# microsoft/XPretrain

Hardware: NVIDIA H100
Metric: video-text pairs/sec (12f x 224^2, 32 tok), CLIP-ViP ViT-B/16 fwd+InfoNCE+bwd (higher is better)
Workload: dtype bf16

## Files before the change

### xpretrain_b200/csrc/attn_wgmma.cuh

```cuda
#pragma once
#include "ptx.cuh"
#include "mma_frag.cuh"

namespace xp {

constexpr int ATILE = 64;
constexpr int ATILE_BYTES = ATILE * 128;
constexpr int STREAM_THREADS = 384;

constexpr int stream_fwd_smem(int stages) { return (2 + 2 * stages) * ATILE_BYTES + 1024 + 64; }
constexpr int stream_kv_smem(int stages) { return (4 + 2 * stages) * ATILE_BYTES + stages * 2 * ATILE * 4 + 1024 + 64; }
constexpr int stream_q_smem(int stages) { return (4 + 2 * stages) * ATILE_BYTES + 1024 + 64; }

__device__ __forceinline__ uint64_t kdesc(uint32_t addr) { return make_smem_desc_sw128(addr, 16, 1024); }
__device__ __forceinline__ uint64_t mndesc(uint32_t addr) { return make_smem_desc_sw128(addr, 8192, 1024); }

__device__ __forceinline__ void acc_to_afrag(const float (&x)[32], uint32_t (&a)[4][4]) {
#pragma unroll
  for (int ks = 0; ks < 4; ++ks) {
    a[ks][0] = pack_bf16(x[8 * ks + 0], x[8 * ks + 1]);
    a[ks][1] = pack_bf16(x[8 * ks + 2], x[8 * ks + 3]);
    a[ks][2] = pack_bf16(x[8 * ks + 4], x[8 * ks + 5]);
    a[ks][3] = pack_bf16(x[8 * ks + 6], x[8 * ks + 7]);
  }
}

template <class Live>
__device__ __forceinline__ void fwd_step(uint32_t sQ, uint32_t sK, uint32_t sV, float (&o)[32], float (&m_run)[2],
                                         float (&l_run)[2], Live live, bool partial = true) {
  const int lane = threadIdx.x & 31, q_lo = ((threadIdx.x >> 5) & 3) * 16 + (lane >> 2);
  float s[32];
#pragma unroll
  for (int i = 0; i < 32; ++i) s[i] = 0.f;
  wgmma_fence_regs(s);
  wgmma_fence();
#pragma unroll
  for (int ks = 0; ks < 4; ++ks) wgmma_m64n64k16_ss<0, 0>(s, kdesc(sQ + ks * 32), kdesc(sK + ks * 32));
  wgmma_commit();
  wgmma_wait<0>();
  wgmma_fence_regs(s);
  if (partial) {
#pragma unroll
    for (int i = 0; i < 8; ++i)
#pragma unroll
      for (int e = 0; e < 4; ++e)
        if (!live(q_lo + (e >> 1) * 8, i * 8 + (lane & 3) * 2 + (e & 1))) s[4 * i + e] = -INFINITY;
  }
// ... 30 lines not shown
    for (int j = 0; j < 4; ++j)
      pl[ks][j] = pack_bf16(s[8 * ks + 2 * j] - bf16_lo(ph[ks][j]), s[8 * ks + 2 * j + 1] - bf16_hi(ph[ks][j]));
  wgmma_fence_regs(o);
  wgmma_fence();
#pragma unroll
  for (int ks = 0; ks < 4; ++ks) {
    const uint64_t vd = mndesc(sV + ks * 16 * 128);
    wgmma_m64n64k16_rs<1>(o, ph[ks], vd);
    wgmma_m64n64k16_rs<1>(o, pl[ks], vd);
  }
  wgmma_commit();
  wgmma_wait<0>();
  wgmma_fence_regs(o);
}

__device__ __forceinline__ void quad_sum(float (&l_run)[2]) {
#pragma unroll
  for (int r = 0; r < 2; ++r) {
    l_run[r] += __shfl_xor_sync(0xffffffffu, l_run[r], 1);
    l_run[r] += __shfl_xor_sync(0xffffffffu, l_run[r], 2);
  }
}

template <class Live>
__device__ __forceinline__ void kv_step(uint32_t sK, uint32_t sV, uint32_t sQ, uint32_t sdO, const float* s_lse,
                                        const float* s_delta, float (&dk)[32], float (&dv)[32], Live live) {
  const int lane = threadIdx.x & 31, k_lo = ((threadIdx.x >> 5) & 3) * 16 + (lane >> 2);
  float st[32], dpt[32];
#pragma unroll
  for (int i = 0; i < 32; ++i) st[i] = dpt[i] = 0.f;
  wgmma_fence_regs(st);
  wgmma_fence_regs(dpt);
  wgmma_fence();
#pragma unroll
  for (int ks = 0; ks < 4; ++ks) {
    wgmma_m64n64k16_ss<0, 0>(st, kdesc(sK + ks * 32), kdesc(sQ + ks * 32));
    wgmma_m64n64k16_ss<0, 0>(dpt, kdesc(sV + ks * 32), kdesc(sdO + ks * 32));
  }
  wgmma_commit();
  wgmma_wait<0>();
  wgmma_fence_regs(st);
  wgmma_fence_regs(dpt);
#pragma unroll
  for (int i = 0; i < 8; ++i)
#pragma unroll
    for (int e = 0; e < 4; ++e) {
      const int q = i * 8 + (lane & 3) * 2 + (e & 1);
      const float p = live(q, k_lo + (e >> 1) * 8) ? fast_exp2(fmaf(st[4 * i + e], LOG2E, -s_lse[q])) : 0.f;
      st[4 * i + e] = p;
      dpt[4 * i + e] = p * (dpt[4 * i + e] - s_delta[q]);
    }
  uint32_t ap[4][4], ad[4][4];
  acc_to_afrag(st, ap);
  acc_to_afrag(dpt, ad);
  wgmma_fence_regs(dv);
  wgmma_fence_regs(dk);
  wgmma_fence();
#pragma unroll
  for (int ks = 0; ks < 4; ++ks) {
    wgmma_m64n64k16_rs<1>(dv, ap[ks], mndesc(sdO + ks * 16 * 128));
    wgmma_m64n64k16_rs<1>(dk, ad[ks], mndesc(sQ + ks * 16 * 128));
  }
  wgmma_commit();
  wgmma_wait<0>();
  wgmma_fence_regs(dv);
  wgmma_fence_regs(dk);
}

template <class Live>
__device__ __forceinline__ void q_step(uint32_t sQ, uint32_t sdO, uint32_t sK, uint32_t sV, const float (&lse_r)[2],
                                       const float (&del_r)[2], float (&dq)[32], Live live) {
  const int lane = threadIdx.x & 31, q_lo = ((threadIdx.x >> 5) & 3) * 16 + (lane >> 2);
  float s[32], dp[32];
#pragma unroll
  for (int i = 0; i < 32; ++i) s[i] = dp[i] = 0.f;
  wgmma_fence_regs(s);
  wgmma_fence_regs(dp);
  wgmma_fence();
#pragma unroll
  for (int ks = 0; ks < 4; ++ks) {
    wgmma_m64n64k16_ss<0, 0>(s, kdesc(sQ + ks * 32), kdesc(sK + ks * 32));
    wgmma_m64n64k16_ss<0, 0>(dp, kdesc(sdO + ks * 32), kdesc(sV + ks * 32));
  }
  wgmma_commit();
  wgmma_wait<0>();
  wgmma_fence_regs(s);
  wgmma_fence_regs(dp);
#pragma unroll
  for (int i = 0; i < 8; ++i)
#pragma unroll
    for (int e = 0; e < 4; ++e) {
      const bool valid = live(q_lo + (e >> 1) * 8, i * 8 + (lane & 3) * 2 + (e & 1));
      const float p = valid ? fast_exp2(fmaf(s[4 * i + e], LOG2E, -lse_r[e >> 1])) : 0.f;
      dp[4 * i + e] = p * (dp[4 * i + e] - del_r[e >> 1]);
    }
  uint32_t ad[4][4];
  acc_to_afrag(dp, ad);
  wgmma_fence_regs(dq);
  wgmma_fence();
#pragma unroll
  for (int ks = 0; ks < 4; ++ks) wgmma_m64n64k16_rs<1>(dq, ad[ks], mndesc(sK + ks * 16 * 128));
  wgmma_commit();
  wgmma_wait<0>();
  wgmma_fence_regs(dq);
}

template <int STAGES>
__device__ __forceinline__ void init_ring(uint64_t* q_full, uint64_t* full, uint64_t* empty, uint32_t full_count,
                                          int nlive, const CUtensorMap* tm0, const CUtensorMap* tm1) {
  if (threadIdx.x == 0) {
    tma_prefetch_desc(tm0);
    tma_prefetch_desc(tm1);
    mbar_init(q_full, 1);
#pragma unroll
    for (int s = 0; s < STAGES; ++s) {
      mbar_init(&full[s], full_count);
      mbar_init(&empty[s], 4 * nlive);
    }
    fence_barrier_init();
  }
  __syncthreads();
}
__device__ __forceinline__ void release_stage(uint64_t* empty, int s) {
  __syncwarp();
// ... 197 lines not shown
```

### xpretrain_b200/csrc/common.cu

```cuda
#include "common.h"

#include <mutex>

#include "../../include/xpretrain_b200.h"

namespace xp {

static thread_local std::string t_error;
std::atomic<int64_t> g_launches{0};

void set_error(const std::string& msg) { t_error = msg; }
int fail(const std::string& msg) {
  t_error = msg;
  return -1;
}

int sm_count() {
  static int cached[64] = {0};
  int dev = 0;
  if (cudaGetDevice(&dev) != cudaSuccess || dev < 0 || dev >= 64) return 132;
  if (cached[dev] == 0) {
    int n = 0;
    if (cudaDeviceGetAttribute(&n, cudaDevAttrMultiProcessorCount, dev) != cudaSuccess || n <= 0) n = 132;
    cached[dev] = n;
// ... 76 lines not shown
                  CU_TENSOR_MAP_FLOAT_OOB_FILL_NONE);
  if (r != CUDA_SUCCESS) return fail("cuTensorMapEncodeTiled failed with CUresult " + std::to_string(int(r)));
  return 0;
}

int make_tmap_bf16_3d(CUtensorMap* out, const void* base, uint64_t inner, uint64_t mid, uint64_t outer,
                      uint64_t row_stride, uint64_t mid_stride, uint32_t box_inner, uint32_t box_mid) {
  EncodeTiledFn fn = encode_fn();
  if (!fn) return fail("cuTensorMapEncodeTiled unavailable (no CUDA driver / no GPU): this library has no CPU path");
  if (!aligned(base, 16)) return fail("tensor map: base pointer must be 16-byte aligned");
  if ((row_stride * 2) % 16 != 0 || (mid_stride * 2) % 16 != 0)
    return fail("tensor map: strides must be multiples of 8 bf16 elements");
  cuuint64_t dims[3] = {inner, mid, outer};
  cuuint64_t strides[2] = {row_stride * 2, mid_stride * 2};
  cuuint32_t box[3] = {box_inner, box_mid, 1};
  cuuint32_t estr[3] = {1, 1, 1};
  CUresult r = fn(out, CU_TENSOR_MAP_DATA_TYPE_BFLOAT16, 3, const_cast<void*>(base), dims, strides, box, estr,
                  CU_TENSOR_MAP_INTERLEAVE_NONE, CU_TENSOR_MAP_SWIZZLE_128B, CU_TENSOR_MAP_L2_PROMOTION_L2_256B,
                  CU_TENSOR_MAP_FLOAT_OOB_FILL_NONE);
  if (r != CUDA_SUCCESS) return fail("cuTensorMapEncodeTiled failed with CUresult " + std::to_string(int(r)));
  return 0;
}

}

extern "C" {
int xp_version(void) { return XP_ABI_VERSION; }
const char* xp_last_error(void) { return xp::t_error.c_str(); }
int64_t xp_launch_count(void) { return xp::g_launches.load(); }
void xp_launch_count_reset(void) { xp::g_launches.store(0); }
}
```

### xpretrain_b200/csrc/common.h

```cpp
#pragma once
#include <cuda.h>
#include <cuda_bf16.h>
#include <cuda_fp16.h>
#include <cuda_runtime.h>
#include <stdint.h>

#include <atomic>
#include <string>
#include <type_traits>

#include "../../include/xpretrain_b200.h"

namespace xp {

void set_error(const std::string& msg);
int fail(const std::string& msg);
extern std::atomic<int64_t> g_launches;
inline void count_launch(int n = 1) { g_launches.fetch_add(n, std::memory_order_relaxed); }

int sm_count();

int make_tmap_bf16_2d(CUtensorMap* out, const void* base, uint64_t inner, uint64_t outer, uint64_t row_stride,
                      uint32_t box_inner, uint32_t box_outer);
int make_tmap_bf16_3d(CUtensorMap* out, const void* base, uint64_t inner, uint64_t mid, uint64_t outer,
                      uint64_t row_stride, uint64_t mid_stride, uint32_t box_inner, uint32_t box_mid);

int ensure_context(const void* device_ptr);
#define XP_ENTER(ptr)                                   \
  do {                                                  \
    if (::xp::ensure_context(ptr) != 0) return -1;      \
  } while (0)

#define XP_CHECK_CUDA(expr)                                                                         \
  do {                                                                                              \
    cudaError_t _e = (expr);                                                                        \
    if (_e != cudaSuccess) return ::xp::fail(std::string(#expr) + ": " + cudaGetErrorString(_e)); \
  } while (0)

#define XP_CHECK_LAUNCH(name)                                                                             \
  do {                                                                                                    \
    cudaError_t _e = cudaGetLastError();                                                                  \
    if (_e != cudaSuccess) return ::xp::fail(std::string(name) + " launch: " + cudaGetErrorString(_e)); \
    ::xp::count_launch();                                                                                 \
  } while (0)

inline bool aligned(const void* p, uintptr_t bytes) { return (reinterpret_cast<uintptr_t>(p) & (bytes - 1)) == 0; }

template <auto K>
// ... 25 lines not shown
```

### xpretrain_b200/csrc/ptx.cuh

```cuda
#pragma once
#include <cuda.h>
#include <cuda_bf16.h>
#include <cuda_fp16.h>
#include <cuda_runtime.h>
#include <stdint.h>
#include <stdio.h>

namespace xp {

#ifndef XP_WAIT_TIMEOUT_CYCLES
#define XP_WAIT_TIMEOUT_CYCLES (8000000000ll)
#endif

__device__ __forceinline__ uint32_t smem_u32(const void* p) {
  return static_cast<uint32_t>(__cvta_generic_to_shared(p));
}
__device__ __forceinline__ int lane_id() { return threadIdx.x & 31; }

__device__ __forceinline__ void mbar_init(uint64_t* bar, uint32_t count) {
  asm volatile("mbarrier.init.shared::cta.b64 [%0], %1;" ::"r"(smem_u32(bar)), "r"(count) : "memory");
}
__device__ __forceinline__ void fence_barrier_init() {
  asm volatile("fence.mbarrier_init.release.cluster;" ::: "memory");
}
// ... 33 lines not shown
}
__device__ __forceinline__ void mbar_wait_nocall(uint64_t* bar, uint32_t parity) {
  if (mbar_try_wait(bar, parity)) return;
  long long t0 = clock64();
  while (!mbar_try_wait(bar, parity)) {
    if (clock64() - t0 > XP_WAIT_TIMEOUT_CYCLES) __trap();
  }
}

__device__ __forceinline__ void tma_prefetch_desc(const CUtensorMap* m) {
  asm volatile("prefetch.tensormap [%0];" ::"l"(reinterpret_cast<uint64_t>(m)) : "memory");
}
__device__ __forceinline__ void tma_load_2d(void* smem_dst, const CUtensorMap* m, uint64_t* bar, int c0, int c1) {
  asm volatile(
      "cp.async.bulk.tensor.2d.shared::cluster.global.mbarrier::complete_tx::bytes [%0], [%1, {%3, %4}], [%2];"
      ::"r"(smem_u32(smem_dst)), "l"(reinterpret_cast<uint64_t>(m)), "r"(smem_u32(bar)), "r"(c0), "r"(c1)
      : "memory");
}
__device__ __forceinline__ void tma_load_3d(void* smem_dst, const CUtensorMap* m, uint64_t* bar, int c0, int c1,
                                            int c2) {
  asm volatile(
      "cp.async.bulk.tensor.3d.shared::cluster.global.mbarrier::complete_tx::bytes [%0], [%1, {%3, %4, %5}], [%2];"
      ::"r"(smem_u32(smem_dst)), "l"(reinterpret_cast<uint64_t>(m)), "r"(smem_u32(bar)), "r"(c0), "r"(c1), "r"(c2)
      : "memory");
}

__device__ __forceinline__ void tma_store_2d(const CUtensorMap* m, uint32_t smem_src, int c0, int c1) {
  asm volatile("cp.async.bulk.tensor.2d.global.shared::cta.bulk_group [%0, {%2, %3}], [%1];" ::"l"(
                   reinterpret_cast<uint64_t>(m)),
               "r"(smem_src), "r"(c0), "r"(c1)
               : "memory");
}
__device__ __forceinline__ void tma_store_commit() { asm volatile("cp.async.bulk.commit_group;" ::: "memory"); }
template <int N>
__device__ __forceinline__ void tma_store_wait_read() {
  asm volatile("cp.async.bulk.wait_group.read %0;" ::"n"(N) : "memory");
}

__device__ __forceinline__ void wgmma_fence() { asm volatile("wgmma.fence.sync.aligned;" ::: "memory"); }
__device__ __forceinline__ void wgmma_commit() { asm volatile("wgmma.commit_group.sync.aligned;" ::: "memory"); }
template <int N>
__device__ __forceinline__ void wgmma_wait() {
  asm volatile("wgmma.wait_group.sync.aligned %0;" ::"n"(N) : "memory");
}
template <int R>
__device__ __forceinline__ void wgmma_fence_regs(float (&d)[R]) {
// ... 14 lines not shown
        "+f"(d[8]), "+f"(d[9]), "+f"(d[10]), "+f"(d[11]), "+f"(d[12]), "+f"(d[13]), "+f"(d[14]), "+f"(d[15]),
        "+f"(d[16]), "+f"(d[17]), "+f"(d[18]), "+f"(d[19]), "+f"(d[20]), "+f"(d[21]), "+f"(d[22]), "+f"(d[23]),
        "+f"(d[24]), "+f"(d[25]), "+f"(d[26]), "+f"(d[27]), "+f"(d[28]), "+f"(d[29]), "+f"(d[30]), "+f"(d[31]),
        "+f"(d[32]), "+f"(d[33]), "+f"(d[34]), "+f"(d[35]), "+f"(d[36]), "+f"(d[37]), "+f"(d[38]), "+f"(d[39]),
        "+f"(d[40]), "+f"(d[41]), "+f"(d[42]), "+f"(d[43]), "+f"(d[44]), "+f"(d[45]), "+f"(d[46]), "+f"(d[47]),
        "+f"(d[48]), "+f"(d[49]), "+f"(d[50]), "+f"(d[51]), "+f"(d[52]), "+f"(d[53]), "+f"(d[54]), "+f"(d[55]),
        "+f"(d[56]), "+f"(d[57]), "+f"(d[58]), "+f"(d[59]), "+f"(d[60]), "+f"(d[61]), "+f"(d[62]), "+f"(d[63])
      : "l"(adesc), "l"(bdesc), "n"(TA), "n"(TB));
}

template <int TA, int TB>
__device__ __forceinline__ void wgmma_m64n64k16_ss(float (&d)[32], uint64_t adesc, uint64_t bdesc) {
  asm volatile(
      "wgmma.mma_async.sync.aligned.m64n64k16.f32.bf16.bf16 {"
      "%0, %1, %2, %3, %4, %5, %6, %7, %8, %9, %10, %11, %12, %13, %14, %15, "
      "%16, %17, %18, %19, %20, %21, %22, %23, %24, %25, %26, %27, %28, %29, %30, %31"
      "}, %32, %33, 1, 1, 1, %34, %35;"
      : "+f"(d[0]), "+f"(d[1]), "+f"(d[2]), "+f"(d[3]), "+f"(d[4]), "+f"(d[5]), "+f"(d[6]), "+f"(d[7]),
        "+f"(d[8]), "+f"(d[9]), "+f"(d[10]), "+f"(d[11]), "+f"(d[12]), "+f"(d[13]), "+f"(d[14]), "+f"(d[15]),
        "+f"(d[16]), "+f"(d[17]), "+f"(d[18]), "+f"(d[19]), "+f"(d[20]), "+f"(d[21]), "+f"(d[22]), "+f"(d[23]),
        "+f"(d[24]), "+f"(d[25]), "+f"(d[26]), "+f"(d[27]), "+f"(d[28]), "+f"(d[29]), "+f"(d[30]), "+f"(d[31])
      : "l"(adesc), "l"(bdesc), "n"(TA), "n"(TB));
}
template <int TB>
__device__ __forceinline__ void wgmma_m64n64k16_rs(float (&d)[32], const uint32_t (&a)[4], uint64_t bdesc) {
  asm volatile(
      "wgmma.mma_async.sync.aligned.m64n64k16.f32.bf16.bf16 {"
      "%0, %1, %2, %3, %4, %5, %6, %7, %8, %9, %10, %11, %12, %13, %14, %15, "
      "%16, %17, %18, %19, %20, %21, %22, %23, %24, %25, %26, %27, %28, %29, %30, %31"
      "}, {%32, %33, %34, %35}, %36, 1, 1, 1, %37;"
      : "+f"(d[0]), "+f"(d[1]), "+f"(d[2]), "+f"(d[3]), "+f"(d[4]), "+f"(d[5]), "+f"(d[6]), "+f"(d[7]),
        "+f"(d[8]), "+f"(d[9]), "+f"(d[10]), "+f"(d[11]), "+f"(d[12]), "+f"(d[13]), "+f"(d[14]), "+f"(d[15]),
        "+f"(d[16]), "+f"(d[17]), "+f"(d[18]), "+f"(d[19]), "+f"(d[20]), "+f"(d[21]), "+f"(d[22]), "+f"(d[23]),
        "+f"(d[24]), "+f"(d[25]), "+f"(d[26]), "+f"(d[27]), "+f"(d[28]), "+f"(d[29]), "+f"(d[30]), "+f"(d[31])
      : "r"(a[0]), "r"(a[1]), "r"(a[2]), "r"(a[3]), "l"(bdesc), "n"(TB));
}

template <uint32_t N>
__device__ __forceinline__ void setmaxnreg_dec() {
  asm volatile("setmaxnreg.dec.sync.aligned.u32 %0;" ::"n"(N));
}
template <uint32_t N>
__device__ __forceinline__ void setmaxnreg_inc() {
  asm volatile("setmaxnreg.inc.sync.aligned.u32 %0;" ::"n"(N));
}
__device__ __forceinline__ void named_bar_sync(uint32_t id, uint32_t threads) {
// ... 130 lines not shown
```

### xpretrain_b200/csrc/vip_attention.cu

```cuda
#include "../../include/xpretrain_b200.h"
#include "common.h"
#include "attn_wgmma.cuh"
#include "vip_attention.h"

namespace xp {

constexpr int SROWS = 256;
constexpr int GROW = 248;
constexpr int MAT_BYTES = SROWS * 128;
constexpr int TILE_BYTES = 64 * 128;
constexpr int ATT_THREADS = 256;

__device__ __forceinline__ bool row_valid(int r, const AttnDims& d) { return r < d.L || (r >= GROW && r < GROW + d.M); }
__device__ __forceinline__ bool row_global(int r) { return r >= GROW; }
__device__ __forceinline__ int row_seq(int r, const AttnDims& d) { return r >= GROW ? r - GROW : d.M + r; }
__device__ __forceinline__ bool tile_live(int k, const AttnDims& d) { return k == 3 || 64 * k < d.L; }

template <int NMAT>
__device__ __forceinline__ void stage_rows(uint8_t* sm, uint64_t* bar, const CUtensorMap* const (&mapL)[NMAT],
                                           const CUtensorMap* const (&mapM)[NMAT], const int (&col)[NMAT], const AttnDims& d,
                                           int b, int t) {
  if (threadIdx.x == 0) {
    mbar_init(bar, 1);
    fence_barrier_init();
// ... 79 lines not shown
}

__global__ void __launch_bounds__(64)
vip_attn_fwd_combine_kernel(const float* __restrict__ part, __nv_bfloat16* __restrict__ out, float* __restrict__ lse,
                            const AttnDims d) {
  const int h = blockIdx.x, b = blockIdx.y, c = threadIdx.x;
  for (int m = 0; m < d.M; ++m) {
    const float* p0 = part + ((static_cast<long long>(b) * d.H + h) * d.T * d.M + m) * 66;
    float mx = -INFINITY;
    for (int t = 0; t < d.T; ++t) mx = fmaxf(mx, p0[static_cast<long long>(t) * d.M * 66]);
    float l = 0.f, acc = 0.f;
    for (int t = 0; t < d.T; ++t) {
      const float* p = p0 + static_cast<long long>(t) * d.M * 66;
      const float w = __expf(p[0] - mx);
      l += p[1] * w;
      acc += p[2 + c] * w;
    }
    out[(static_cast<long long>(b) * d.S + m) * d.ld_o + h * HD + c] = __float2bfloat16(acc / l);
    if (c == 0) lse[(static_cast<long long>(b) * d.H + h) * d.S + m] = mx + logf(l);
  }
}


__global__ void __launch_bounds__(ATT_THREADS, 1)
vip_attn_bwd_kernel(const __grid_constant__ CUtensorMap tmL, const __grid_constant__ CUtensorMap tmM,
                    const __grid_constant__ CUtensorMap tdL, const __grid_constant__ CUtensorMap tdM,
                    const __nv_bfloat16* __restrict__ out, const __nv_bfloat16* __restrict__ dout, const float* __restrict__ lse,
                    __nv_bfloat16* __restrict__ dqkv, float* __restrict__ gpart, const AttnDims d, float q_scale) {
  extern __shared__ uint8_t smem_raw[];
  uint8_t* sm = smem_raw + (((smem_u32(smem_raw) + 1023u) & ~1023u) - smem_u32(smem_raw));
  float* s_lse = reinterpret_cast<float*>(sm + 4 * MAT_BYTES);
  float* s_delta = s_lse + SROWS;
  uint64_t* bar = reinterpret_cast<uint64_t*>(s_delta + SROWS);
  const int t = blockIdx.x, h = blockIdx.y, b = blockIdx.z;
  {
    const CUtensorMap* const mL[4] = {&tmL, &tmL, &tmL, &tdL};
    const CUtensorMap* const mM[4] = {&tmM, &tmM, &tmM, &tdM};
    const int col[4] = {h * HD, d.C + h * HD, 2 * d.C + h * HD, h * HD};
    stage_rows<4>(sm, bar, mL, mM, col, d, b, t);
  }
  for (int base = 0; base < SROWS; base += ATT_THREADS / 8) {
    const int row = base + (threadIdx.x >> 3), chunk = threadIdx.x & 7;
    float dot = 0.f;
    const bool valid = row_valid(row, d);
    long long tr = 0;
    if (valid) {
      tr = token_row(d, b, t, row_seq(row, d));
      const long long off = tr * d.ld_o + h * HD + chunk * 8;
      const uint4 g = *reinterpret_cast<const uint4*>(dout + off);
      const uint4 o = *reinterpret_cast<const uint4*>(out + off);
      const uint32_t gw[4] = {g.x, g.y, g.z, g.w}, ow[4] = {o.x, o.y, o.z, o.w};
#pragma unroll
      for (int i = 0; i < 4; ++i) dot += bf16_lo(gw[i]) * bf16_lo(ow[i]) + bf16_hi(gw[i]) * bf16_hi(ow[i]);
    }
    dot += __shfl_xor_sync(0xffffffffu, dot, 1);
    dot += __shfl_xor_sync(0xffffffffu, dot, 2);
    dot += __shfl_xor_sync(0xffffffffu, dot, 4);
    if (chunk == 0) {
      s_delta[row] = dot;
      s_lse[row] = valid ? lse[(static_cast<long long>(b) * d.H + h) * d.S + (tr - static_cast<long long>(b) * d.S)] * LOG2E
                         : INFINITY;
    }
  }
  __syncthreads();

  const uint32_t sQ = smem_u32(sm), sK = sQ + MAT_BYTES, sV = sK + MAT_BYTES, sdO = sV + MAT_BYTES;
  const int wg = threadIdx.x >> 7, wq = (threadIdx.x >> 5) & 3, lane = threadIdx.x & 31;
  const bool mask_gg = (t != 0);
  const auto pair_live = [&](int q, int key) {
    return row_valid(q, d) && row_valid(key, d) && !(mask_gg && row_global(q) && row_global(key));
  };
  float* gp = gpart + ((static_cast<long long>(b) * d.H + h) * d.T + t) * d.M * 3 * HD;

  for (int kt = wg; kt < 4; kt += 2) {
    if (!tile_live(kt, d)) continue;
    const int k_lo = kt * 64 + wq * 16 + (lane >> 2);
    float dk[32], dv[32];
#pragma unroll
    for (int i = 0; i < 32; ++i) dk[i] = dv[i] = 0.f;
#pragma unroll 1
    for (int qb = 0; qb < 4; ++qb) {
      if (!tile_live(qb, d)) continue;
      kv_step(sK + kt * TILE_BYTES, sV + kt * TILE_BYTES, sQ + qb * TILE_BYTES, sdO + qb * TILE_BYTES, s_lse + qb * 64,
              s_delta + qb * 64, dk, dv, [&](int q, int key) { return pair_live(qb * 64 + q, kt * 64 + key); });
    }
#pragma unroll
    for (int r = 0; r < 2; ++r) {
      const int key = k_lo + r * 8;
      if (!row_valid(key, d)) continue;
      if (!row_global(key)) {
        __nv_bfloat16* row = dqkv + token_row(d, b, t, row_seq(key, d)) * d.ld_qkv + h * HD + (lane & 3) * 2;
#pragma unroll
        for (int i = 0; i < 8; ++i) {
          *reinterpret_cast<uint32_t*>(row + d.C + i * 8) = pack_bf16(dk[4 * i + 2 * r], dk[4 * i + 2 * r + 1]);
          *reinterpret_cast<uint32_t*>(row + 2 * d.C + i * 8) = pack_bf16(dv[4 * i + 2 * r], dv[4 * i + 2 * r + 1]);
        }
      } else {
        float* g = gp + static_cast<long long>(key - GROW) * 3 * HD + (lane & 3) * 2;
#pragma unroll
        for (int i = 0; i < 8; ++i) {
          g[HD + i * 8] = dk[4 * i + 2 * r]; g[HD + i * 8 + 1] = dk[4 * i + 2 * r + 1];
          g[2 * HD + i * 8] = dv[4 * i + 2 * r]; g[2 * HD + i * 8 + 1] = dv[4 * i + 2 * r + 1];
        }
      }
    }
  }

  for (int qt = wg; qt < 4; qt += 2) {
    if (!tile_live(qt, d)) continue;
    const int q_lo = qt * 64 + wq * 16 + (lane >> 2);
    const float lse_r[2] = {s_lse[q_lo], s_lse[q_lo + 8]}, del_r[2] = {s_delta[q_lo], s_delta[q_lo + 8]};
    float dq[32];
#pragma unroll
    for (int i = 0; i < 32; ++i) dq[i] = 0.f;
#pragma unroll 1
    for (int kb = 0; kb < 4; ++kb) {
      if (!tile_live(kb, d)) continue;
      q_step(sQ + qt * TILE_BYTES, sdO + qt * TILE_BYTES, sK + kb * TILE_BYTES, sV + kb * TILE_BYTES, lse_r, del_r, dq,
             [&](int q, int key) { return pair_live(qt * 64 + q, kb * 64 + key); });
    }
#pragma unroll
    for (int r = 0; r < 2; ++r) {
      const int q = q_lo + r * 8;
      if (!row_valid(q, d)) continue;
      if (!row_global(q)) {
        __nv_bfloat16* row = dqkv + token_row(d, b, t, row_seq(q, d)) * d.ld_qkv + h * HD + (lane & 3) * 2;
#pragma unroll
        for (int i = 0; i < 8; ++i)
          *reinterpret_cast<uint32_t*>(row + i * 8) = pack_bf16(dq[4 * i + 2 * r] * q_scale, dq[4 * i + 2 * r + 1] * q_scale);
      } else {
        float* g = gp + static_cast<long long>(q - GROW) * 3 * HD + (lane & 3) * 2;
#pragma unroll
        for (int i = 0; i < 8; ++i) {
          g[i * 8] = dq[4 * i + 2 * r];
          g[i * 8 + 1] = dq[4 * i + 2 * r + 1];
        }
      }
    }
  }
}

__global__ void __launch_bounds__(192)
vip_attn_bwd_combine_kernel(const float* __restrict__ gpart, __nv_bfloat16* __restrict__ dqkv, const AttnDims d,
                            float q_scale) {
  const int h = blockIdx.x, b = blockIdx.y;
  const int which = threadIdx.x / HD, c = threadIdx.x % HD;
  for (int m = 0; m < d.M; ++m) {
    float acc = 0.f;
    for (int t = 0; t < d.T; ++t)
      acc += gpart[((((static_cast<long long>(b) * d.H + h) * d.T + t) * d.M + m) * 3 + which) * HD + c];
    if (which == 0) acc *= q_scale;
    dqkv[(static_cast<long long>(b) * d.S + m) * d.ld_qkv + static_cast<long long>(which) * d.C + h * HD + c] =
        __float2bfloat16(acc);
  }
}


static int make_dims(AttnDims& d, int B, int H, int T, int L, int M, int C) {
  if (C != H * HD) return fail("vip_attention: head_dim must be 64 (C == 64*H)");
  if (L < 1) return fail("vip_attention: L must be >= 1");
  if (M < 1 || M > 8) return fail("vip_attention: 1 <= M <= 8 global tokens");
  d.B = B; d.H = H; d.T = T; d.L = L; d.M = M;
  d.S = static_cast<long long>(M) + static_cast<long long>(T) * L;
  d.C = C;
  d.ld_qkv = 3LL * C;
  d.ld_o = C;
  return 0;
}

static int make_row_maps(CUtensorMap* mL, CUtensorMap* mM, const void* base, long long width, const AttnDims& d) {
  const uint64_t rows = static_cast<uint64_t>(d.B) * static_cast<uint64_t>(d.S);
  if (make_tmap_bf16_2d(mL, base, width, rows, width, HD, d.L)) return -1;
  return make_tmap_bf16_2d(mM, base, width, rows, width, HD, d.M);
}

constexpr int FWD_SMEM = 3 * MAT_BYTES + 1024 + 64;
constexpr int BWD_SMEM = 4 * MAT_BYTES + 2 * SROWS * 4 + 1024 + 64;

}

using namespace xp;

extern "C" int64_t xp_vip_attention_workspace_bytes(int32_t B, int32_t H, int32_t T, int32_t M) {
  return static_cast<int64_t>(B) * H * T * M * 3 * HD * sizeof(float);
}

extern "C" int xp_vip_attention_fwd(const void* qkv, void* out, float* lse, float* workspace, int32_t B, int32_t H,
                                    int32_t T, int32_t L, int32_t M, int32_t C, void* stream) {
  XP_ENTER(qkv);
  AttnDims d;
  if (make_dims(d, B, H, T, L, M, C)) return -1;
  cudaStream_t st = static_cast<cudaStream_t>(stream);
  if (M + L > VIP_STAGED_MAX_ROWS) {
    if (vip_long_attn_fwd(d, qkv, out, lse, workspace, st)) return -1;
  } else {
    CUtensorMap mL, mM;
    if (make_row_maps(&mL, &mM, qkv, 3LL * C, d)) return -1;
    if (smem_limit<vip_attn_fwd_kernel>(FWD_SMEM)) return -1;
    vip_attn_fwd_kernel<<<dim3(T, H, B), ATT_THREADS, FWD_SMEM, st>>>(mL, mM, static_cast<__nv_bfloat16*>(out), lse, workspace, d);
    XP_CHECK_LAUNCH("vip_attn_fwd_kernel");
  }
  vip_attn_fwd_combine_kernel<<<dim3(H, B), 64, 0, st>>>(workspace, static_cast<__nv_bfloat16*>(out), lse, d);
  XP_CHECK_LAUNCH("vip_attn_fwd_combine_kernel");
  return 0;
}

extern "C" int xp_vip_attention_bwd(const void* qkv, const void* out, const void* dout, const float* lse, void* dqkv,
                                    float* workspace, int32_t B, int32_t H, int32_t T, int32_t L, int32_t M, int32_t C,
                                    float q_scale, void* stream) {
  XP_ENTER(qkv);
  AttnDims d;
  if (make_dims(d, B, H, T, L, M, C)) return -1;
  cudaStream_t st = static_cast<cudaStream_t>(stream);
  if (M + L > VIP_STAGED_MAX_ROWS) {
    if (vip_long_attn_bwd(d, qkv, out, dout, lse, dqkv, workspace, q_scale, st)) return -1;
  } else {
    CUtensorMap mL, mM, gL, gM;
    if (make_row_maps(&mL, &mM, qkv, 3LL * C, d) || make_row_maps(&gL, &gM, dout, C, d)) return -1;
    if (smem_limit<vip_attn_bwd_kernel>(BWD_SMEM)) return -1;
    vip_attn_bwd_kernel<<<dim3(T, H, B), ATT_THREADS, BWD_SMEM, st>>>(
        mL, mM, gL, gM, static_cast<const __nv_bfloat16*>(out), static_cast<const __nv_bfloat16*>(dout), lse,
        static_cast<__nv_bfloat16*>(dqkv), workspace, d, q_scale);
    XP_CHECK_LAUNCH("vip_attn_bwd_kernel");
  }
  vip_attn_bwd_combine_kernel<<<dim3(H, B), 192, 0, st>>>(workspace, static_cast<__nv_bfloat16*>(dqkv), d, q_scale);
  XP_CHECK_LAUNCH("vip_attn_bwd_combine_kernel");
  return 0;
}
```

Baseline: 288.2.

## Make ViP attention backward a persistent warp-specialized kernel with TMA slot pipelining

Replaces the one-CTA-per-(t,h,b) backward kernel with a persistent grid of at most one CTA per SM. One producer warpgroup issues 4D/3D TMA loads into a double-buffered slot ring and computes delta/lse, while two consumer warpgroups run the dK/dV and dQ wgmma steps. Rows are packed tightly (frame rows plus global rows padded to 8), so tile count follows L. A trailing short tile uses n16 wgmma instead of n64. The intent is to overlap loads with compute, cut padded MMA work and amortize launch/prologue cost. The price is mbarrier/register-reallocation complexity, and there is a single slot when shared memory is tight.

```diff
diff --git a/xpretrain_b200/csrc/attn_wgmma.cuh b/xpretrain_b200/csrc/attn_wgmma.cuh
--- a/xpretrain_b200/csrc/attn_wgmma.cuh
+++ b/xpretrain_b200/csrc/attn_wgmma.cuh
@@ -15,14 +15,22 @@
 __device__ __forceinline__ uint64_t kdesc(uint32_t addr) { return make_smem_desc_sw128(addr, 16, 1024); }
 __device__ __forceinline__ uint64_t mndesc(uint32_t addr) { return make_smem_desc_sw128(addr, 8192, 1024); }
 
-__device__ __forceinline__ void acc_to_afrag(const float (&x)[32], uint32_t (&a)[4][4]) {
-#pragma unroll
-  for (int ks = 0; ks < 4; ++ks) {
+template <int R>
+__device__ __forceinline__ void acc_to_afrag(const float (&x)[R], uint32_t (&a)[R / 8][4]) {
+#pragma unroll
+  for (int ks = 0; ks < R / 8; ++ks) {
     a[ks][0] = pack_bf16(x[8 * ks + 0], x[8 * ks + 1]);
     a[ks][1] = pack_bf16(x[8 * ks + 2], x[8 * ks + 3]);
     a[ks][2] = pack_bf16(x[8 * ks + 4], x[8 * ks + 5]);
     a[ks][3] = pack_bf16(x[8 * ks + 6], x[8 * ks + 7]);
   }
+}
+
+template <int N>
+__device__ __forceinline__ void wgmma_ss(float (&d)[N / 2], uint64_t adesc, uint64_t bdesc) {
+  static_assert(N == 64 || N == 16, "block width");
+  if constexpr (N == 64) wgmma_m64n64k16_ss<0, 0>(d, adesc, bdesc);
+  else wgmma_m64n16k16_ss<0, 0>(d, adesc, bdesc);
 }
 
 template <class Live>
@@ -99,27 +107,27 @@
   }
 }
 
-template <class Live>
+template <int N = 64, class Live>
 __device__ __forceinline__ void kv_step(uint32_t sK, uint32_t sV, uint32_t sQ, uint32_t sdO, const float* s_lse,
                                         const float* s_delta, float (&dk)[32], float (&dv)[32], Live live) {
   const int lane = threadIdx.x & 31, k_lo = ((threadIdx.x >> 5) & 3) * 16 + (lane >> 2);
-  float st[32], dpt[32];
-#pragma unroll
-  for (int i = 0; i < 32; ++i) st[i] = dpt[i] = 0.f;
+  float st[N / 2], dpt[N / 2];
+#pragma unroll
+  for (int i = 0; i < N / 2; ++i) st[i] = dpt[i] = 0.f;
   wgmma_fence_regs(st);
   wgmma_fence_regs(dpt);
   wgmma_fence();
 #pragma unroll
   for (int ks = 0; ks < 4; ++ks) {
-    wgmma_m64n64k16_ss<0, 0>(st, kdesc(sK + ks * 32), kdesc(sQ + ks * 32));
-    wgmma_m64n64k16_ss<0, 0>(dpt, kdesc(sV + ks * 32), kdesc(sdO + ks * 32));
+    wgmma_ss<N>(st, kdesc(sK + ks * 32), kdesc(sQ + ks * 32));
+    wgmma_ss<N>(dpt, kdesc(sV + ks * 32), kdesc(sdO + ks * 32));
   }
   wgmma_commit();
   wgmma_wait<0>();
   wgmma_fence_regs(st);
   wgmma_fence_regs(dpt);
 #pragma unroll
-  for (int i = 0; i < 8; ++i)
+  for (int i = 0; i < N / 8; ++i)
 #pragma unroll
     for (int e = 0; e < 4; ++e) {
       const int q = i * 8 + (lane & 3) * 2 + (e & 1);
@@ -127,14 +135,14 @@
       st[4 * i + e] = p;
       dpt[4 * i + e] = p * (dpt[4 * i + e] - s_delta[q]);
     }
-  uint32_t ap[4][4], ad[4][4];
+  uint32_t ap[N / 16][4], ad[N / 16][4];
   acc_to_afrag(st, ap);
   acc_to_afrag(dpt, ad);
   wgmma_fence_regs(dv);
   wgmma_fence_regs(dk);
   wgmma_fence();
 #pragma unroll
-  for (int ks = 0; ks < 4; ++ks) {
+  for (int ks = 0; ks < N / 16; ++ks) {
     wgmma_m64n64k16_rs<1>(dv, ap[ks], mndesc(sdO + ks * 16 * 128));
     wgmma_m64n64k16_rs<1>(dk, ad[ks], mndesc(sQ + ks * 16 * 128));
   }
@@ -144,39 +152,39 @@
   wgmma_fence_regs(dk);
 }
 
-template <class Live>
+template <int N = 64, class Live>
 __device__ __forceinline__ void q_step(uint32_t sQ, uint32_t sdO, uint32_t sK, uint32_t sV, const float (&lse_r)[2],
                                        const float (&del_r)[2], float (&dq)[32], Live live) {
   const int lane = threadIdx.x & 31, q_lo = ((threadIdx.x >> 5) & 3) * 16 + (lane >> 2);
-  float s[32], dp[32];
-#pragma unroll
-  for (int i = 0; i < 32; ++i) s[i] = dp[i] = 0.f;
+  float s[N / 2], dp[N / 2];
+#pragma unroll
+  for (int i = 0; i < N / 2; ++i) s[i] = dp[i] = 0.f;
   wgmma_fence_regs(s);
   wgmma_fence_regs(dp);
   wgmma_fence();
 #pragma unroll
   for (int ks = 0; ks < 4; ++ks) {
-    wgmma_m64n64k16_ss<0, 0>(s, kdesc(sQ + ks * 32), kdesc(sK + ks * 32));
-    wgmma_m64n64k16_ss<0, 0>(dp, kdesc(sdO + ks * 32), kdesc(sV + ks * 32));
+    wgmma_ss<N>(s, kdesc(sQ + ks * 32), kdesc(sK + ks * 32));
+    wgmma_ss<N>(dp, kdesc(sdO + ks * 32), kdesc(sV + ks * 32));
   }
   wgmma_commit();
   wgmma_wait<0>();
   wgmma_fence_regs(s);
   wgmma_fence_regs(dp);
 #pragma unroll
-  for (int i = 0; i < 8; ++i)
+  for (int i = 0; i < N / 8; ++i)
 #pragma unroll
     for (int e = 0; e < 4; ++e) {
       const bool valid = live(q_lo + (e >> 1) * 8, i * 8 + (lane & 3) * 2 + (e & 1));
       const float p = valid ? fast_exp2(fmaf(s[4 * i + e], LOG2E, -lse_r[e >> 1])) : 0.f;
       dp[4 * i + e] = p * (dp[4 * i + e] - del_r[e >> 1]);
     }
-  uint32_t ad[4][4];
+  uint32_t ad[N / 16][4];
   acc_to_afrag(dp, ad);
   wgmma_fence_regs(dq);
   wgmma_fence();
 #pragma unroll
-  for (int ks = 0; ks < 4; ++ks) wgmma_m64n64k16_rs<1>(dq, ad[ks], mndesc(sK + ks * 16 * 128));
+  for (int ks = 0; ks < N / 16; ++ks) wgmma_m64n64k16_rs<1>(dq, ad[ks], mndesc(sK + ks * 16 * 128));
   wgmma_commit();
   wgmma_wait<0>();
   wgmma_fence_regs(dq);
diff --git a/xpretrain_b200/csrc/common.cu b/xpretrain_b200/csrc/common.cu
--- a/xpretrain_b200/csrc/common.cu
+++ b/xpretrain_b200/csrc/common.cu
@@ -122,6 +122,24 @@
   return 0;
 }
 
+int make_tmap_bf16_4d(CUtensorMap* out, const void* base, uint64_t inner, uint64_t d1, uint64_t d2, uint64_t d3,
+                      uint64_t stride1, uint64_t stride2, uint64_t stride3, uint32_t box_inner, uint32_t box_d1) {
+  EncodeTiledFn fn = encode_fn();
+  if (!fn) return fail("cuTensorMapEncodeTiled unavailable (no CUDA driver / no GPU): this library has no CPU path");
+  if (!aligned(base, 16)) return fail("tensor map: base pointer must be 16-byte aligned");
+  if ((stride1 * 2) % 16 != 0 || (stride2 * 2) % 16 != 0 || (stride3 * 2) % 16 != 0)
+    return fail("tensor map: strides must be multiples of 8 bf16 elements");
+  cuuint64_t dims[4] = {inner, d1, d2, d3};
+  cuuint64_t strides[3] = {stride1 * 2, stride2 * 2, stride3 * 2};
+  cuuint32_t box[4] = {box_inner, box_d1, 1, 1};
+  cuuint32_t estr[4] = {1, 1, 1, 1};
+  CUresult r = fn(out, CU_TENSOR_MAP_DATA_TYPE_BFLOAT16, 4, const_cast<void*>(base), dims, strides, box, estr,
+                  CU_TENSOR_MAP_INTERLEAVE_NONE, CU_TENSOR_MAP_SWIZZLE_128B, CU_TENSOR_MAP_L2_PROMOTION_L2_256B,
+                  CU_TENSOR_MAP_FLOAT_OOB_FILL_NONE);
+  if (r != CUDA_SUCCESS) return fail("cuTensorMapEncodeTiled failed with CUresult " + std::to_string(int(r)));
+  return 0;
+}
+
 }
 
 extern "C" {
diff --git a/xpretrain_b200/csrc/common.h b/xpretrain_b200/csrc/common.h
--- a/xpretrain_b200/csrc/common.h
+++ b/xpretrain_b200/csrc/common.h
@@ -24,6 +24,8 @@
                       uint32_t box_inner, uint32_t box_outer);
 int make_tmap_bf16_3d(CUtensorMap* out, const void* base, uint64_t inner, uint64_t mid, uint64_t outer,
                       uint64_t row_stride, uint64_t mid_stride, uint32_t box_inner, uint32_t box_mid);
+int make_tmap_bf16_4d(CUtensorMap* out, const void* base, uint64_t inner, uint64_t d1, uint64_t d2, uint64_t d3,
+                      uint64_t stride1, uint64_t stride2, uint64_t stride3, uint32_t box_inner, uint32_t box_d1);
 
 int ensure_context(const void* device_ptr);
 #define XP_ENTER(ptr)                                   \
diff --git a/xpretrain_b200/csrc/ptx.cuh b/xpretrain_b200/csrc/ptx.cuh
--- a/xpretrain_b200/csrc/ptx.cuh
+++ b/xpretrain_b200/csrc/ptx.cuh
@@ -79,6 +79,15 @@
   asm volatile(
       "cp.async.bulk.tensor.3d.shared::cluster.global.mbarrier::complete_tx::bytes [%0], [%1, {%3, %4, %5}], [%2];"
       ::"r"(smem_u32(smem_dst)), "l"(reinterpret_cast<uint64_t>(m)), "r"(smem_u32(bar)), "r"(c0), "r"(c1), "r"(c2)
+      : "memory");
+}
+
+__device__ __forceinline__ void tma_load_4d(void* smem_dst, const CUtensorMap* m, uint64_t* bar, int c0, int c1,
+                                            int c2, int c3) {
+  asm volatile(
+      "cp.async.bulk.tensor.4d.shared::cluster.global.mbarrier::complete_tx::bytes [%0], [%1, {%3, %4, %5, %6}], [%2];"
+      ::"r"(smem_u32(smem_dst)), "l"(reinterpret_cast<uint64_t>(m)), "r"(smem_u32(bar)), "r"(c0), "r"(c1), "r"(c2),
+        "r"(c3)
       : "memory");
 }
 
@@ -139,6 +148,14 @@
         "+f"(d[24]), "+f"(d[25]), "+f"(d[26]), "+f"(d[27]), "+f"(d[28]), "+f"(d[29]), "+f"(d[30]), "+f"(d[31])
       : "l"(adesc), "l"(bdesc), "n"(TA), "n"(TB));
 }
+template <int TA, int TB>
+__device__ __forceinline__ void wgmma_m64n16k16_ss(float (&d)[8], uint64_t adesc, uint64_t bdesc) {
+  asm volatile(
+      "wgmma.mma_async.sync.aligned.m64n16k16.f32.bf16.bf16 {"
+      "%0, %1, %2, %3, %4, %5, %6, %7}, %8, %9, 1, 1, 1, %10, %11;"
+      : "+f"(d[0]), "+f"(d[1]), "+f"(d[2]), "+f"(d[3]), "+f"(d[4]), "+f"(d[5]), "+f"(d[6]), "+f"(d[7])
+      : "l"(adesc), "l"(bdesc), "n"(TA), "n"(TB));
+}
 template <int TB>
 __device__ __forceinline__ void wgmma_m64n64k16_rs(float (&d)[32], const uint32_t (&a)[4], uint64_t bdesc) {
   asm volatile(
diff --git a/xpretrain_b200/csrc/vip_attention.cu b/xpretrain_b200/csrc/vip_attention.cu
--- a/xpretrain_b200/csrc/vip_attention.cu
+++ b/xpretrain_b200/csrc/vip_attention.cu
@@ -125,121 +125,223 @@
 }
 
 
-__global__ void __launch_bounds__(ATT_THREADS, 1)
+constexpr int BWD_THREADS = 384;
+constexpr int BWD_STAT = 256;
+
+__host__ __device__ constexpr int bwd_grow(int L) { return (L + 7) & ~7; }
+__host__ __device__ constexpr int bwd_rows(int L) { return bwd_grow(L) + 8; }
+__host__ __device__ constexpr int bwd_tiles(int L) { return (bwd_rows(L) + 63) / 64; }
+__host__ __device__ constexpr int bwd_slot_bytes(int L) { return (3 * bwd_rows(L) + 64 * bwd_tiles(L)) * 128; }
+constexpr int bwd_smem(int L, int nslots) { return nslots * (bwd_slot_bytes(L) + 2 * BWD_STAT * 4 + 3 * 8) + 1024; }
+
+#ifdef XP_VIP_BWD_PHASES
+constexpr int PH_CTAS = 4, PH_ITEMS = 16, PH_STAMPS = 8;
+__device__ long long g_vip_bwd_phases[PH_CTAS * PH_ITEMS * PH_STAMPS];
+#define VIP_BWD_STAMP(i, k)                                                                           \
+  do {                                                                                                \
+    if ((threadIdx.x == 0 || threadIdx.x == 128) && blockIdx.x < PH_CTAS && (i) < PH_ITEMS)           \
+      g_vip_bwd_phases[(blockIdx.x * PH_ITEMS + (i)) * PH_STAMPS + (k)] = clock64();                  \
+  } while (0)
+#else
+#define VIP_BWD_STAMP(i, k) \
+  do {                      \
+  } while (0)
+#endif
+
+__global__ void __launch_bounds__(BWD_THREADS, 1)
 vip_attn_bwd_kernel(const __grid_constant__ CUtensorMap tmL, const __grid_constant__ CUtensorMap tmM,
                     const __grid_constant__ CUtensorMap tdL, const __grid_constant__ CUtensorMap tdM,
-                    const __nv_bfloat16* __restrict__ out, const __nv_bfloat16* __restrict__ dout, const float* __restrict__ lse,
-                    __nv_bfloat16* __restrict__ dqkv, float* __restrict__ gpart, const AttnDims d, float q_scale) {
+                    const __nv_bfloat16* __restrict__ out, const float* __restrict__ lse,
+                    __nv_bfloat16* __restrict__ dqkv, float* __restrict__ gpart, const AttnDims d, float q_scale,
+                    int nslots) {
   extern __shared__ uint8_t smem_raw[];
   uint8_t* sm = smem_raw + (((smem_u32(smem_raw) + 1023u) & ~1023u) - smem_u32(smem_raw));
-  float* s_lse = reinterpret_cast<float*>(sm + 4 * MAT_BYTES);
-  float* s_delta = s_lse + SROWS;
-  uint64_t* bar = reinterpret_cast<uint64_t*>(s_delta + SROWS);
-  const int t = blockIdx.x, h = blockIdx.y, b = blockIdx.z;
-  {
-    const CUtensorMap* const mL[4] = {&tmL, &tmL, &tmL, &tdL};
-    const CUtensorMap* const mM[4] = {&tmM, &tmM, &tmM, &tdM};
-    const int col[4] = {h * HD, d.C + h * HD, 2 * d.C + h * HD, h * HD};
-    stage_rows<4>(sm, bar, mL, mM, col, d, b, t);
-  }
-  for (int base = 0; base < SROWS; base += ATT_THREADS / 8) {
-    const int row = base + (threadIdx.x >> 3), chunk = threadIdx.x & 7;
-    float dot = 0.f;
-    const bool valid = row_valid(row, d);
-    long long tr = 0;
-    if (valid) {
-      tr = token_row(d, b, t, row_seq(row, d));
-      const long long off = tr * d.ld_o + h * HD + chunk * 8;
-      const uint4 g = *reinterpret_cast<const uint4*>(dout + off);
-      const uint4 o = *reinterpret_cast<const uint4*>(out + off);
-      const uint32_t gw[4] = {g.x, g.y, g.z, g.w}, ow[4] = {o.x, o.y, o.z, o.w};
-#pragma unroll
-      for (int i = 0; i < 4; ++i) dot += bf16_lo(gw[i]) * bf16_lo(ow[i]) + bf16_hi(gw[i]) * bf16_hi(ow[i]);
-    }
-    dot += __shfl_xor_sync(0xffffffffu, dot, 1);
-    dot += __shfl_xor_sync(0xffffffffu, dot, 2);
-    dot += __shfl_xor_sync(0xffffffffu, dot, 4);
-    if (chunk == 0) {
-      s_delta[row] = dot;
-      s_lse[row] = valid ? lse[(static_cast<long long>(b) * d.H + h) * d.S + (tr - static_cast<long long>(b) * d.S)] * LOG2E
-                         : INFINITY;
-    }
+  const int G = bwd_grow(d.L), R = bwd_rows(d.L), NT = bwd_tiles(d.L), slot_bytes = bwd_slot_bytes(d.L);
+  float* stats = reinterpret_cast<float*>(sm + nslots * slot_bytes);
+  uint64_t* load = reinterpret_cast<uint64_t*>(stats + nslots * 2 * BWD_STAT);
+  uint64_t* full = load + nslots;
+  uint64_t* empty = full + nslots;
+  const int items = d.B * d.H * d.T;
+  const int wg = threadIdx.x >> 7;
+  if (threadIdx.x == 0) {
+    tma_prefetch_desc(&tmL);
+    tma_prefetch_desc(&tmM);
+    tma_prefetch_desc(&tdL);
+    tma_prefetch_desc(&tdM);
+    for (int s = 0; s < nslots; ++s) {
+      mbar_init(&load[s], 1);
+      mbar_init(&full[s], 128);
+      mbar_init(&empty[s], 8);
+    }
+    fence_barrier_init();
   }
   __syncthreads();
-
-  const uint32_t sQ = smem_u32(sm), sK = sQ + MAT_BYTES, sV = sK + MAT_BYTES, sdO = sV + MAT_BYTES;
-  const int wg = threadIdx.x >> 7, wq = (threadIdx.x >> 5) & 3, lane = threadIdx.x & 31;
-  const bool mask_gg = (t != 0);
-  const auto pair_live = [&](int q, int key) {
-    return row_valid(q, d) && row_valid(key, d) && !(mask_gg && row_global(q) && row_global(key));
-  };
-  float* gp = gpart + ((static_cast<long long>(b) * d.H + h) * d.T + t) * d.M * 3 * HD;
-
-  for (int kt = wg; kt < 4; kt += 2) {
-    if (!tile_live(kt, d)) continue;
-    const int k_lo = kt * 64 + wq * 16 + (lane >> 2);
-    float dk[32], dv[32];
-#pragma unroll
-    for (int i = 0; i < 32; ++i) dk[i] = dv[i] = 0.f;
+  const auto row_ok = [&](int r) { return r < d.L || (r >= G && r < G + d.M); };
+  const auto seq_of = [&](int r) { return r >= G ? r - G : d.M + r; };
+
+  if (wg == 0) {
+    setmaxnreg_dec<40>();
+    const int tid = threadIdx.x, chunk = tid & 7;
+    for (int it = 0, item = blockIdx.x; item < items; ++it, item += gridDim.x) {
+      const int s = it % nslots;
+      const uint32_t ph = (it / nslots) & 1;
+      const int t = item % d.T, h = (item / d.T) % d.H, b = item / (d.T * d.H);
+      uint8_t* slot = sm + s * slot_bytes;
+      if (tid == 0) mbar_wait_nocall(&empty[s], ph ^ 1);
+      named_bar_sync(1, 128);
+      VIP_BWD_STAMP(it, 5);
+      if (tid == 0) {
+        mbar_arrive_expect_tx(&load[s], slot_bytes);
+        const int cq = h * HD;
+#pragma unroll
+        for (int m = 0; m < 3; ++m) {
+          tma_load_4d(slot + m * R * 128, &tmL, &load[s], m * d.C + cq, 0, t, b);
+          tma_load_3d(slot + (m * R + G) * 128, &tmM, &load[s], m * d.C + cq, 0, b);
+        }
+        tma_load_4d(slot + 3 * R * 128, &tdL, &load[s], cq, 0, t, b);
+        tma_load_3d(slot + (3 * R + G) * 128, &tdM, &load[s], cq, 0, b);
+      }
+      float* s_lse = stats + s * 2 * BWD_STAT;
+      const uint32_t sdO = smem_u32(slot) + 3 * R * 128;
+      for (int base = 0; base < 64 * NT; base += 16) {
+        const int row = base + (tid >> 3);
+        const bool valid = row_ok(row);
+        long long tr = 0;
+        uint4 o = make_uint4(0u, 0u, 0u, 0u);
+        float l = INFINITY;
+        if (valid) {
+          tr = token_row(d, b, t, seq_of(row));
+          o = *reinterpret_cast<const uint4*>(out + tr * d.ld_o + h * HD + chunk * 8);
+          l = lse[(static_cast<long long>(b) * d.H + h) * d.S + (tr - static_cast<long long>(b) * d.S)] * LOG2E;
+        }
+        mbar_wait_nocall(&load[s], ph);
+        if (base == 0) VIP_BWD_STAMP(it, 6);
+        uint4 g;
+        asm volatile("ld.shared.v4.u32 {%0, %1, %2, %3}, [%4];"
+                     : "=r"(g.x), "=r"(g.y), "=r"(g.z), "=r"(g.w)
+                     : "r"(sdO + row * 128 + ((chunk ^ (row & 7)) << 4)));
+        const uint32_t gw[4] = {g.x, g.y, g.z, g.w}, ow[4] = {o.x, o.y, o.z, o.w};
+        float dot = 0.f;
+#pragma unroll
+        for (int i = 0; i < 4; ++i) dot += bf16_lo(gw[i]) * bf16_lo(ow[i]) + bf16_hi(gw[i]) * bf16_hi(ow[i]);
+        dot += __shfl_xor_sync(0xffffffffu, dot, 1);
+        dot += __shfl_xor_sync(0xffffffffu, dot, 2);
+        dot += __shfl_xor_sync(0xffffffffu, dot, 4);
+        if (chunk == 0) {
+          s_lse[BWD_STAT + row] = dot;
+          s_lse[row] = l;
+        }
+      }
+      fence_proxy_async_smem();
+      VIP_BWD_STAMP(it, 7);
+      mbar_arrive(&full[s]);
+    }
+    return;
+  }
+
+  setmaxnreg_inc<232>();
+  const int c = wg - 1, wq = (threadIdx.x >> 5) & 3, lane = threadIdx.x & 31;
+  const bool short_last = NT > 1 && R - 64 * (NT - 1) <= 16;
+  for (int it = 0, item = blockIdx.x; item < items; ++it, item += gridDim.x) {
+    const int s = it % nslots;
+    const uint32_t ph = (it / nslots) & 1;
+    const int t = item % d.T, h = (item / d.T) % d.H, b = item / (d.T * d.H);
+    const uint32_t sQ = smem_u32(sm + s * slot_bytes), sK = sQ + R * 128, sV = sK + R * 128, sdO = sV + R * 128;
+    const float* s_lse = stats + s * 2 * BWD_STAT;
+    const float* s_delta = s_lse + BWD_STAT;
+    VIP_BWD_STAMP(it, 0);
+    mbar_wait_nocall(&load[s], ph);
+    VIP_BWD_STAMP(it, 1);
+    mbar_wait_nocall(&full[s], ph);
+    VIP_BWD_STAMP(it, 2);
+    const bool mask_gg = (t != 0);
+    const auto pair_cols = [&](int row, int col) -> uint64_t {
+      const auto below = [](int n) { return n >= 64 ? ~0ull : n <= 0 ? 0ull : (1ull << n) - 1; };
+      if (!row_ok(row)) return 0ull;
+      const int r0 = col * 64;
+      uint64_t m = below(d.L - r0) | (below(G + d.M - r0) & ~below(G - r0));
+      if (mask_gg && row >= G) m &= below(G - r0);
+      return m;
+    };
+    float* gp = gpart + ((static_cast<long long>(b) * d.H + h) * d.T + t) * d.M * 3 * HD;
+
+    for (int kt = c; kt < NT; kt += 2) {
+      const int k_lo = kt * 64 + wq * 16 + (lane >> 2);
+      float dk[32], dv[32];
+#pragma unroll
+      for (int i = 0; i < 32; ++i) dk[i] = dv[i] = 0.f;
 #pragma unroll 1
-    for (int qb = 0; qb < 4; ++qb) {
-      if (!tile_live(qb, d)) continue;
-      kv_step(sK + kt * TILE_BYTES, sV + kt * TILE_BYTES, sQ + qb * TILE_BYTES, sdO + qb * TILE_BYTES, s_lse + qb * 64,
-              s_delta + qb * 64, dk, dv, [&](int q, int key) { return pair_live(qb * 64 + q, kt * 64 + key); });
-    }
-#pragma unroll
-    for (int r = 0; r < 2; ++r) {
-      const int key = k_lo + r * 8;
-      if (!row_valid(key, d)) continue;
-      if (!row_global(key)) {
-        __nv_bfloat16* row = dqkv + token_row(d, b, t, row_seq(key, d)) * d.ld_qkv + h * HD + (lane & 3) * 2;
-#pragma unroll
-        for (int i = 0; i < 8; ++i) {
-          *reinterpret_cast<uint32_t*>(row + d.C + i * 8) = pack_bf16(dk[4 * i + 2 * r], dk[4 * i + 2 * r + 1]);
-          *reinterpret_cast<uint32_t*>(row + 2 * d.C + i * 8) = pack_bf16(dv[4 * i + 2 * r], dv[4 * i + 2 * r + 1]);
-        }
-      } else {
-        float* g = gp + static_cast<long long>(key - GROW) * 3 * HD + (lane & 3) * 2;
-#pragma unroll
-        for (int i = 0; i < 8; ++i) {
-          g[HD + i * 8] = dk[4 * i + 2 * r]; g[HD + i * 8 + 1] = dk[4 * i + 2 * r + 1];
-          g[2 * HD + i * 8] = dv[4 * i + 2 * r]; g[2 * HD + i * 8 + 1] = dv[4 * i + 2 * r + 1];
-        }
-      }
-    }
-  }
-
-  for (int qt = wg; qt < 4; qt += 2) {
-    if (!tile_live(qt, d)) continue;
-    const int q_lo = qt * 64 + wq * 16 + (lane >> 2);
-    const float lse_r[2] = {s_lse[q_lo], s_lse[q_lo + 8]}, del_r[2] = {s_delta[q_lo], s_delta[q_lo + 8]};
-    float dq[32];
-#pragma unroll
-    for (int i = 0; i < 32; ++i) dq[i] = 0.f;
+      for (int qb = 0; qb < NT; ++qb) {
+        const uint64_t live[2] = {pair_cols(k_lo, qb), pair_cols(k_lo + 8, qb)};
+        const auto pred = [&](int q, int key) { return ((live[(key >> 3) & 1] >> q) & 1) != 0; };
+        const uint32_t qo = qb * TILE_BYTES;
+        if (qb == NT - 1 && short_last)
+          kv_step<16>(sK + kt * TILE_BYTES, sV + kt * TILE_BYTES, sQ + qo, sdO + qo, s_lse + qb * 64, s_delta + qb * 64,
+                      dk, dv, pred);
+        else
+          kv_step(sK + kt * TILE_BYTES, sV + kt * TILE_BYTES, sQ + qo, sdO + qo, s_lse + qb * 64, s_delta + qb * 64, dk,
+                  dv, pred);
+      }
+#pragma unroll
+      for (int r = 0; r < 2; ++r) {
+        const int key = k_lo + r * 8;
+        if (!row_ok(key)) continue;
+        if (key < G) {
+          __nv_bfloat16* row = dqkv + token_row(d, b, t, seq_of(key)) * d.ld_qkv + h * HD + (lane & 3) * 2;
+#pragma unroll
+          for (int i = 0; i < 8; ++i) {
+            *reinterpret_cast<uint32_t*>(row + d.C + i * 8) = pack_bf16(dk[4 * i + 2 * r], dk[4 * i + 2 * r + 1]);
+            *reinterpret_cast<uint32_t*>(row + 2 * d.C + i * 8) = pack_bf16(dv[4 * i + 2 * r], dv[4 * i + 2 * r + 1]);
+          }
+        } else {
+          float* g = gp + static_cast<long long>(key - G) * 3 * HD + (lane & 3) * 2;
+#pragma unroll
+          for (int i = 0; i < 8; ++i) {
+            g[HD + i * 8] = dk[4 * i + 2 * r]; g[HD + i * 8 + 1] = dk[4 * i + 2 * r + 1];
+            g[2 * HD + i * 8] = dv[4 * i + 2 * r]; g[2 * HD + i * 8 + 1] = dv[4 * i + 2 * r + 1];
+          }
+        }
+      }
+    }
+    VIP_BWD_STAMP(it, 3);
+
+    for (int qt = c; qt < NT; qt += 2) {
+      const int q_lo = qt * 64 + wq * 16 + (lane >> 2);
+      const float lse_r[2] = {s_lse[q_lo], s_lse[q_lo + 8]}, del_r[2] = {s_delta[q_lo], s_delta[q_lo + 8]};
+      float dq[32];
+#pragma unroll
+      for (int i = 0; i < 32; ++i) dq[i] = 0.f;
 #pragma unroll 1
-    for (int kb = 0; kb < 4; ++kb) {
-      if (!tile_live(kb, d)) continue;
-      q_step(sQ + qt * TILE_BYTES, sdO + qt * TILE_BYTES, sK + kb * TILE_BYTES, sV + kb * TILE_BYTES, lse_r, del_r, dq,
-             [&](int q, int key) { return pair_live(qt * 64 + q, kb * 64 + key); });
-    }
-#pragma unroll
-    for (int r = 0; r < 2; ++r) {
-      const int q = q_lo + r * 8;
-      if (!row_valid(q, d)) continue;
-      if (!row_global(q)) {
-        __nv_bfloat16* row = dqkv + token_row(d, b, t, row_seq(q, d)) * d.ld_qkv + h * HD + (lane & 3) * 2;
-#pragma unroll
-        for (int i = 0; i < 8; ++i)
-          *reinterpret_cast<uint32_t*>(row + i * 8) = pack_bf16(dq[4 * i + 2 * r] * q_scale, dq[4 * i + 2 * r + 1] * q_scale);
-      } else {
-        float* g = gp + static_cast<long long>(q - GROW) * 3 * HD + (lane & 3) * 2;
-#pragma unroll
-        for (int i = 0; i < 8; ++i) {
-          g[i * 8] = dq[4 * i + 2 * r];
-          g[i * 8 + 1] = dq[4 * i + 2 * r + 1];
-        }
-      }
-    }
+      for (int kb = 0; kb < NT; ++kb) {
+        const uint64_t live[2] = {pair_cols(q_lo, kb), pair_cols(q_lo + 8, kb)};
+        const auto pred = [&](int q, int key) { return ((live[(q >> 3) & 1] >> key) & 1) != 0; };
+        const uint32_t ko = kb * TILE_BYTES;
+        if (kb == NT - 1 && short_last)
+          q_step<16>(sQ + qt * TILE_BYTES, sdO + qt * TILE_BYTES, sK + ko, sV + ko, lse_r, del_r, dq, pred);
+        else
+          q_step(sQ + qt * TILE_BYTES, sdO + qt * TILE_BYTES, sK + ko, sV + ko, lse_r, del_r, dq, pred);
+      }
+#pragma unroll
+      for (int r = 0; r < 2; ++r) {
+        const int q = q_lo + r * 8;
+        if (!row_ok(q)) continue;
+        if (q < G) {
+          __nv_bfloat16* row = dqkv + token_row(d, b, t, seq_of(q)) * d.ld_qkv + h * HD + (lane & 3) * 2;
+#pragma unroll
+          for (int i = 0; i < 8; ++i)
+            *reinterpret_cast<uint32_t*>(row + i * 8) = pack_bf16(dq[4 * i + 2 * r] * q_scale, dq[4 * i + 2 * r + 1] * q_scale);
+        } else {
+          float* g = gp + static_cast<long long>(q - G) * 3 * HD + (lane & 3) * 2;
+#pragma unroll
+          for (int i = 0; i < 8; ++i) {
+            g[i * 8] = dq[4 * i + 2 * r];
+            g[i * 8 + 1] = dq[4 * i + 2 * r + 1];
+          }
+        }
+      }
+    }
+    VIP_BWD_STAMP(it, 4);
+    release_stage(empty, s);
   }
 }
 
@@ -277,8 +379,16 @@
   return make_tmap_bf16_2d(mM, base, width, rows, width, HD, d.M);
 }
 
+static int make_bwd_maps(CUtensorMap* mL, CUtensorMap* mM, const void* base, long long width, const AttnDims& d,
+                         int gbox) {
+  const auto* frames = static_cast<const __nv_bfloat16*>(base) + d.M * width;
+  if (make_tmap_bf16_4d(mL, frames, width, d.L, d.T, d.B, width, d.L * width, d.S * width, HD, bwd_grow(d.L)))
+    return -1;
+  return make_tmap_bf16_3d(mM, base, width, d.M, d.B, width, d.S * width, HD, gbox);
+}
+
 constexpr int FWD_SMEM = 3 * MAT_BYTES + 1024 + 64;
-constexpr int BWD_SMEM = 4 * MAT_BYTES + 2 * SROWS * 4 + 1024 + 64;
+constexpr int BWD_SMEM_MAX = 227 * 1024;
 
 }
 
@@ -319,14 +429,29 @@
     if (vip_long_attn_bwd(d, qkv, out, dout, lse, dqkv, workspace, q_scale, st)) return -1;
   } else {
     CUtensorMap mL, mM, gL, gM;
-    if (make_row_maps(&mL, &mM, qkv, 3LL * C, d) || make_row_maps(&gL, &gM, dout, C, d)) return -1;
-    if (smem_limit<vip_attn_bwd_kernel>(BWD_SMEM)) return -1;
-    vip_attn_bwd_kernel<<<dim3(T, H, B), ATT_THREADS, BWD_SMEM, st>>>(
-        mL, mM, gL, gM, static_cast<const __nv_bfloat16*>(out), static_cast<const __nv_bfloat16*>(dout), lse,
-        static_cast<__nv_bfloat16*>(dqkv), workspace, d, q_scale);
+    if (make_bwd_maps(&mL, &mM, qkv, 3LL * C, d, 8) ||
+        make_bwd_maps(&gL, &gM, dout, C, d, 64 * bwd_tiles(L) - bwd_grow(L)))
+      return -1;
+    if (smem_limit<vip_attn_bwd_kernel>(BWD_SMEM_MAX)) return -1;
+    const int nslots = bwd_smem(L, 2) <= BWD_SMEM_MAX ? 2 : 1;
+    const int items = B * H * T;
+    vip_attn_bwd_kernel<<<items < sm_count() ? items : sm_count(), BWD_THREADS, bwd_smem(L, nslots), st>>>(
+        mL, mM, gL, gM, static_cast<const __nv_bfloat16*>(out), lse, static_cast<__nv_bfloat16*>(dqkv), workspace, d,
+        q_scale, nslots);
     XP_CHECK_LAUNCH("vip_attn_bwd_kernel");
   }
   vip_attn_bwd_combine_kernel<<<dim3(H, B), 192, 0, st>>>(workspace, static_cast<__nv_bfloat16*>(dqkv), d, q_scale);
   XP_CHECK_LAUNCH("vip_attn_bwd_combine_kernel");
   return 0;
 }
+
+#ifdef XP_VIP_BWD_PHASES
+extern "C" int xp_vip_attention_bwd_phases(int64_t* host) {
+  XP_CHECK_CUDA(cudaDeviceSynchronize());
+  XP_CHECK_CUDA(cudaMemcpyFromSymbol(host, g_vip_bwd_phases, sizeof(g_vip_bwd_phases)));
+  void* dev = nullptr;
+  XP_CHECK_CUDA(cudaGetSymbolAddress(&dev, g_vip_bwd_phases));
+  XP_CHECK_CUDA(cudaMemset(dev, 0, sizeof(g_vip_bwd_phases)));
+  return 0;
+}
+#endif
```

New measurement: 299.7, median of 6. +4.0%, better.
